# manikya7022/Continual-Learning-for-Dynamic-Video-Quality-Enhancement

Measured on AMD Instinct MI355X. Metric: train frames/sec (2x SR, T=3, 540p->1080p), higher is better.
Workload: dtype bf16

## Files before the change

continual-learning-for-dynamic-video-quality-enhancement_amd/csrc/conv_bf16.hip:

```cpp
#include "conv_common.h"

namespace nvq {

#ifdef NVQ_DEBUG_TOOLS
static int g_debug_mode = 0;
void set_conv_debug_mode(int m) { g_debug_mode = m; }
#else
constexpr int g_debug_mode = 0;
#endif

constexpr int XSB = 48;

__device__ __forceinline__ __bf16 pack_bf16_elem(const float* __restrict__ w, int cout_w, int cin_w, int taps, int transpose,
                                                 int cout_keep, int NT, int nkc, long idx) {
    const int stride = ws_stride_halfs(taps, NT);
    long t = idx % stride;
    const long slab = idx / stride;
    if (t >= (long)taps * 4 * NT * 8) return (__bf16)0.f;
    const int j = t & 7; t >>= 3;
    const int n = t % NT; t /= NT;
    const int g = t & 3; t >>= 2;
    const int tap = (int)t;
    const int kc = slab % nkc;
    const int cz = (int)(slab / nkc);
// ... 721 lines not shown
            for (int k = 0; k < XPER; ++k) {
                const int item = rtid + k * 256;
                *reinterpret_cast<u32x4*>(xs + (item >> 2) * XSB + 8 * (item & 3)) = xok[k] ? xr[k] : z;
            }
        }
        __syncthreads();
        if (kc + 1 < nkc && !(dbg & 4)) fetch(kc + 1);
        if (dbg & 2) continue;
        bf16x8 px[4];
        px[0] = ldP(1, 0, 1); px[1] = ldP(1, 1, 1); px[2] = ldP(2, 0, 1); px[3] = ldP(2, 1, 1);
#pragma unroll
        for (int cb = 0; cb < NBL; ++cb) {
            const bf16x8 wf = ldL(cb);
#pragma unroll
            for (int pb = 0; pb < 4; ++pb)
                lacc[cb][pb] = __builtin_amdgcn_mfma_f32_16x16x32_bf16(wf, px[pb], lacc[cb][pb], 0, 0, 0);
        }
    }
    bool okp[4];
    uint2 rr[4][NBL];
    float4 bb[NBL];
    const __bf16* r16 = reinterpret_cast<const __bf16*>(dl.res) + dl.res_coff;
    auto res_load = [&](int pb) {
        const int gy = ty * TH + 2 * w4 + (pb >> 1), gx = tx * TW + (pb & 1) * 16 + c;
        okp[pb] = gy < H && gx < W;
        const unsigned off = okp[pb] ? ((unsigned)(n * H + gy) * (unsigned)W + gx) * (unsigned)dl.res_ld + 4u * g : 0u;
#pragma unroll
        for (int cb = 0; cb < NBL; ++cb) rr[pb][cb] = *reinterpret_cast<const uint2*>(r16 + (off + cb * 16u));
    };
    if (!(dbg & 128)) { res_load(0); res_load(1); }
    __syncthreads();
    __syncthreads();
    {
        const __bf16* t4 = ws;
#pragma unroll
        for (int cb = 0; cb < NBL; ++cb) {
            const bf16x8 wf = ldL(cb);
#pragma unroll
            for (int pb = 0; pb < 4; ++pb) {
                const int px = (2 * w4 + (pb >> 1)) * TW + (pb & 1) * 16 + c;
                const bf16x8 yf = *reinterpret_cast<const bf16x8*>(t4 + px * T4S + 8 * g);
                lacc[cb][pb] = __builtin_amdgcn_mfma_f32_16x16x32_bf16(wf, yf, lacc[cb][pb], 0, 0, 0);
            }
        }
    }
    if (!(dbg & 128)) { res_load(2); res_load(3); }
#pragma unroll
    for (int cb = 0; cb < NBL; ++cb) bb[cb] = ld4(dl.bias + cb * 16 + 4 * g);
    __syncthreads();
    __bf16* stage = lds + w4 * (2 * TW * STAGE_PX64);
#pragma unroll
    for (int pb = 0; pb < 4; ++pb) {
        if (!okp[pb]) continue;
#pragma unroll
        for (int cb = 0; cb < NBL; ++cb) {
            float v[4] = {lacc[cb][pb][0] + bb[cb].x, lacc[cb][pb][1] + bb[cb].y, lacc[cb][pb][2] + bb[cb].z,
                          lacc[cb][pb][3] + bb[cb].w};
            {
#pragma clang fp contract(off)
                v[0] = v[0] * dl.alpha + __uint_as_float(rr[pb][cb].x << 16);
                v[1] = v[1] * dl.alpha + __uint_as_float(rr[pb][cb].x & 0xffff0000u);
                v[2] = v[2] * dl.alpha + __uint_as_float(rr[pb][cb].y << 16);
                v[3] = v[3] * dl.alpha + __uint_as_float(rr[pb][cb].y & 0xffff0000u);
            }
            *reinterpret_cast<bf16x4*>(stage + ((pb >> 1) * TW + (pb & 1) * 16 + c) * STAGE_PX64 + cb * 16 + 4 * g) =
                (bf16x4){(__bf16)v[0], (__bf16)v[1], (__bf16)v[2], (__bf16)v[3]};
        }
    }
    __builtin_amdgcn_fence(__ATOMIC_RELEASE, "wavefront");
    __builtin_amdgcn_wave_barrier();
    if (dbg & 16) return;
    __bf16* o16 = reinterpret_cast<__bf16*>(dl.out);
#pragma unroll
    for (int k = 0; k < 8; ++k) {
        const int item = lane + k * 64;
        const int px = item >> 3, piece = item & 7;
        const int gy = ty * TH + 2 * w4 + (px >> 5), gx = tx * TW + (px & 31);
        if (gy < H && gx < W)
            *reinterpret_cast<u32x4*>(o16 + ((size_t)(n * H + gy) * W + gx) * dl.out_ld + dl.out_coff + 8 * piece) =
                *reinterpret_cast<const u32x4*>(stage + px * STAGE_PX64 + 8 * piece);
    }
}

template <int KS, bool XB, bool YB, int CIC, int COC = 32>
__global__ __launch_bounds__(256, 2) void wgrad_bf16_kernel(const nvq_wgrad_desc d, int tilesX, int tilesY,
                                                             int ntiles, int nci32, int nco) {
    static_assert(CIC == 32 || (CIC == 64 && XB), "64-channel chunks need bf16 x");
    static_assert(COC == 32 || (COC == 64 && CIC == 64 && YB && KS == 1), "64-co chunks: 1x1, bf16 x and dy");
    constexpr int HALO = KS / 2;
    constexpr int TAPS = KS * KS;
    constexpr int HW_ = TW + 2 * HALO;
    constexpr int HH_ = TH + 2 * HALO;
    constexpr int NPIX = HW_ * HH_;
    constexpr int XSX = CIC == 64 ? 80 : XSB;
    constexpr int XPP = (XB ? 4 : 8) * (CIC / 32);
    constexpr int YSX = COC == 64 ? 80 : XSB;
    constexpr int YPP = (YB ? 4 : 8) * (COC / 32);
    constexpr int XCH = CIC / XPP, YCH = COC / YPP;
    constexpr int XITEMS = NPIX * XPP;
    constexpr int XPER = (XITEMS + 255) / 256;
    constexpr int YPER = TH * TW * YPP / 256;
    constexpr int NCO = (CIC == 64 ? 2 : 1) * (COC / 32);
    __shared__ __attribute__((aligned(16))) __bf16 lds[NPIX * XSX + TH * TW * YSX];
    __bf16* xs = lds;
    __bf16* dys = lds + NPIX * XSX;

    const int tid = threadIdx.x;
    const int lane = tid & 63;
    const int wave = tid >> 6;
    const int r = lane & 15;
    const int g = lane >> 4;
    const int q = r >> 2, p = r & 3;
    const int cib = CIC == 64 ? wave : wave >> 1;
    const int cob0 = CIC == 64 ? 0 : (wave & 1);
    const int cic = blockIdx.y, coc = blockIdx.z;
    const int H = d.h, W = d.w;
    const float* x32 = d.x + d.x_coff;
    const __bf16* x16 = reinterpret_cast<const __bf16*>(d.x) + d.x_coff;
    const float* dy32 = d.dy + d.dy_coff;
    const __bf16* dy16 = reinterpret_cast<const __bf16*>(d.dy) + d.dy_coff;

    f32x4 acc[NCO][TAPS];
#pragma unroll
    for (int a = 0; a < NCO; ++a)
#pragma unroll
        for (int t = 0; t < TAPS; ++t) acc[a][t] = (f32x4){0.f, 0.f, 0.f, 0.f};

    u32x4 xr[XPER], yr[YPER];
    float4 bsumA = make_float4(0.f, 0.f, 0.f, 0.f), bsumB = bsumA;
    const int xq = XCH * (tid & (XPP - 1));
    const int yq = YCH * (tid & (YPP - 1));
    const bool xch_ok = cic * CIC + xq < d.cin;
    const int xch = cic * CIC + xq;
    const bool xlead = !d.x_plane || xch < d.x_ld;
    const unsigned xmul = xlead ? d.x_ld : 32;
    const size_t xbase = xlead ? (size_t)xch : (size_t)(xch >> 5) * d.x_plane + (xch & 31);
    const int ych = coc * COC + yq;
    const bool ych_ok = ych < d.cout;
    unsigned xmask = 0, ymask = 0;
    auto fetch = [&](int tile) {
        int bt = xcd_tile(tile, ntiles);
        const int tx = bt % tilesX; bt /= tilesX;
        const int ty = bt % tilesY;
        const int n = bt / tilesY;
        xmask = 0; ymask = 0;
#pragma unroll
        for (int k = 0; k < XPER; ++k) {
            const int item = tid + k * 256;
            const int hp = item / XPP;
            const int hy = hp / HW_, hx = hp - hy * HW_;
            const int gy = ty * TH + hy - HALO, gx = tx * TW + hx - HALO;
            const bool ok = item < XITEMS && gy >= 0 && gy < H && gx >= 0 && gx < W && xch_ok;
            xmask |= (ok ? 1u : 0u) << k;
            const size_t off = ok ? ((size_t)(n * H + gy) * W + gx) * xmul + xbase : 0;
            if constexpr (XB) xr[k] = *reinterpret_cast<const u32x4*>(x16 + off);
            else xr[k] = *reinterpret_cast<const u32x4*>(x32 + off);
        }
#pragma unroll
        for (int k = 0; k < YPER; ++k) {
            const int item = tid + k * 256;
            const int pp = item / YPP;
            const int py = pp / TW, px = pp - py * TW;
            const int gy = ty * TH + py, gx = tx * TW + px;
            const bool ok = gy < H && gx < W && ych_ok;
            ymask |= (ok ? 1u : 0u) << k;
            const size_t off = ok ? ((size_t)(n * H + gy) * W + gx) * d.dy_ld + ych : 0;
            if constexpr (YB) yr[k] = *reinterpret_cast<const u32x4*>(dy16 + off);
            else yr[k] = *reinterpret_cast<const u32x4*>(dy32 + off);
        }
    };
    auto commit = [&]() {
        const u32x4 z = {0u, 0u, 0u, 0u};
#pragma unroll
        for (int k = 0; k < XPER; ++k) {
            const int item = tid + k * 256;
            if (item < XITEMS) {
                const u32x4 v = (xmask >> k) & 1 ? xr[k] : z;
                __bf16* dst = xs + (item / XPP) * XSX + XCH * (item & (XPP - 1));
                if constexpr (XB) *reinterpret_cast<u32x4*>(dst) = v;
                else *reinterpret_cast<bf16x4*>(dst) = cvt4(as_f4(v));
            }
        }
#pragma unroll
        for (int k = 0; k < YPER; ++k) {
            const int item = tid + k * 256;
            const u32x4 v = (ymask >> k) & 1 ? yr[k] : z;
            __bf16* dst = dys + (item / YPP) * YSX + YCH * (item & (YPP - 1));
            if constexpr (YB) {
                *reinterpret_cast<u32x4*>(dst) = v;
                bsumA.x += bf_lo(v[0]); bsumA.y += bf_hi(v[0]); bsumA.z += bf_lo(v[1]); bsumA.w += bf_hi(v[1]);
                bsumB.x += bf_lo(v[2]); bsumB.y += bf_hi(v[2]); bsumB.z += bf_lo(v[3]); bsumB.w += bf_hi(v[3]);
            } else {
                const float4 f = as_f4(v);
                *reinterpret_cast<bf16x4*>(dst) = cvt4(f);
                bsumA.x += f.x; bsumA.y += f.y; bsumA.z += f.z; bsumA.w += f.w;
            }
        }
    };
    const bool idle = cic * CIC + cib * 16 >= d.cin_w;
    typedef s16x4 __attribute__((address_space(3))) * lds_s16x4_ptr;
    auto tr_read = [&](const __bf16* base, int stride, int pix, int chblock) -> s16x4 {
        return __builtin_amdgcn_ds_read_tr16_b64_v4i16((lds_s16x4_ptr)(base + (pix + q) * stride + chblock * 16 + 4 * p));
    };

    int tile = blockIdx.x;
    if (tile < ntiles) fetch(tile);
    for (; tile < ntiles; tile += gridDim.x) {
        __syncthreads();
        commit();
        __syncthreads();
        if (tile + (int)gridDim.x < ntiles) fetch(tile + gridDim.x);
        if (idle) continue;
#pragma unroll 2
        for (int py = 0; py < TH; ++py) {
            bf16x8 bfrag[NCO];
#pragma unroll
            for (int a = 0; a < NCO; ++a) {
                const s16x4 b0 = tr_read(dys, YSX, py * TW + 4 * g, cob0 + a);
                const s16x4 b1 = tr_read(dys, YSX, py * TW + 16 + 4 * g, cob0 + a);
                bfrag[a] = __builtin_bit_cast(bf16x8, __builtin_shufflevector(b0, b1, 0, 1, 2, 3, 4, 5, 6, 7));
            }
#pragma unroll
            for (int tap = 0; tap < TAPS; ++tap) {
                const int ddy = tap / KS, ddx = tap - ddy * KS;
                const int hp = (py + ddy) * HW_ + ddx;
                const s16x4 a0 = tr_read(xs, XSX, hp + 4 * g, cib);
                const s16x4 a1 = tr_read(xs, XSX, hp + 16 + 4 * g, cib);
                const bf16x8 afrag = __builtin_bit_cast(bf16x8, __builtin_shufflevector(a0, a1, 0, 1, 2, 3, 4, 5, 6, 7));
#pragma unroll
                for (int a = 0; a < NCO; ++a)
                    acc[a][tap] = __builtin_amdgcn_mfma_f32_16x16x32_bf16(afrag, bfrag[a], acc[a][tap], 0, 0, 0);
            }
        }
    }

    const int slab = cic * (CIC / 32) + (cib * 16) / 32;
    if (slab < nci32) {
        const int cil0 = (cib * 16) % 32;
#pragma unroll
        for (int a = 0; a < NCO; ++a) {
            const int coc32 = coc * (COC / 32) + (cob0 + a) / 2, cob = (cob0 + a) % 2;
            if (coc32 >= nco) continue;
            float* part = d.workspace + ((size_t)(blockIdx.x * nci32 + slab) * nco + coc32) * (TAPS * WG_C * WG_C);
#pragma unroll
            for (int tap = 0; tap < TAPS; ++tap)
#pragma unroll
                for (int e = 0; e < 4; ++e) part[(tap * WG_C + cil0 + 4 * g + e) * WG_C + cob * 16 + r] = acc[a][tap][e];
        }
    }

    if (cic == 0 && d.dbias != nullptr) {
        float* scratch = reinterpret_cast<float*>(lds);
        __syncthreads();
        st4(scratch + 8 * tid, bsumA);
        st4(scratch + 8 * tid + 4, bsumB);
        __syncthreads();
        if (tid < COC) {
            const int piece = tid / YCH, e = tid % YCH;
            float s = 0.f;
            for (int k = 0; k < 256 / YPP; ++k) s += scratch[8 * (YPP * k + piece) + e];
            float* bp = d.workspace + (size_t)WGRAD_MAX_SLABS * 9 * WG_C * WG_C;
            const int coc32 = coc * (COC / 32) + tid / WG_C;
            if (coc32 < nco) bp[((size_t)blockIdx.x * nco + coc32) * WG_C + tid % WG_C] = s;
        }
    }
}

size_t pack_floats_bf16(int cout, int cin_store, int ksize) {
    const int NT = choose_nt(cout);
    const size_t ncz = (cout + NT - 1) / NT, nkc = (cin_store + KCB - 1) / KCB;
    return ncz * nkc * (size_t)ws_stride_halfs(ksize * ksize, NT) / 2;
}

int pack_bf16(const float* w, int cout_w, int cin_w, int ksize, int transpose, int cin_store, int cout_keep,
              float* wpack, hipStream_t s) {
    const int cout = transpose ? cout_keep : cout_w;
    const int NT = choose_nt(cout);
    const int ncz = (cout + NT - 1) / NT, nkc = (cin_store + KCB - 1) / KCB;
    const long total = (long)ncz * nkc * ws_stride_halfs(ksize * ksize, NT);
    int nblk = ceil_div(total, 256);
    if (nblk > 2048) nblk = 2048;
    hipLaunchKernelGGL(pack_bf16_kernel, dim3(nblk), dim3(256), 0, s, w, cout_w, cin_w, ksize * ksize, transpose,
                       cout_keep, NT, ncz, nkc, reinterpret_cast<__bf16*>(wpack));
    return check_launch("conv_pack_bf16");
}

PackJobDev pack_job_bf16(const nvq_pack_job& j) {
    const int cout = j.transpose ? j.cout_keep : j.cout_w;
    const int NT = choose_nt(cout);
    const int ncz = (cout + NT - 1) / NT, nkc = (j.cin_store + KCB - 1) / KCB;
    return PackJobDev{j.w, j.wpack, j.cout_w, j.cin_w, j.ksize * j.ksize, j.transpose, j.cout_keep, NT, ncz, nkc,
                      (long)ncz * nkc * ws_stride_halfs(j.ksize * j.ksize, NT)};
}

int pack_batch_bf16(const PackJobTable& t, int n, hipStream_t s) {
    hipLaunchKernelGGL(pack_batch_bf16_kernel, dim3(32, n), dim3(256), 0, s, t);
    return check_launch("conv_pack_batch(bf16)");
}

int conv_forward_bf16(const nvq_conv_desc& d, int vec_ok, hipStream_t s) {
    NVQ_REQUIRE((size_t)d.n * d.h * d.w * d.in_ld < ((size_t)1 << 32),
                "conv_forward(bf16): input tensor of %d x %d x %d x %d elements exceeds the 32-bit offsets of the kernels", d.n,
                d.h, d.w, d.in_ld);
    const int NT = choose_nt(d.cout);
    const int ncz = (d.cout_store + NT - 1) / NT;
    const int nkc = (d.cin + KCB - 1) / KCB;
    int tilesX = (d.w + TW - 1) / TW, tilesY = (d.h + TH - 1) / TH;
    const bool underfilled = tilesX * ((d.h + 2 * TH - 1) / (2 * TH)) < NVQ_SMALL_IMAGE_TILES;
    const int rows = d.tile_rows == 0 && underfilled ? 8 : d.tile_rows;
    if (d.ksize == 3 && NT == 32 && d.in_bf16 && d.h >= 2 * TH && vec_ok &&
        (rows == 162 || rows == 164 || (rows == 0 && d.cin <= 128)))
        return conv_forward_m32(d, rows == 164 ? 4 : 2, g_debug_mode & 15, s);
    if (d.ksize == 3 && NT == 32 && d.in_bf16 && d.h >= 2 * TH && rows != 8) {
        tilesY = (d.h + 2 * TH - 1) / (2 * TH);
        const dim3 grid8((unsigned)((long)tilesX * tilesY * d.n), ncz);
        hipLaunchKernelGGL((conv_bf16_kernel<2, 3, true, 8>), grid8, dim3(512), 0, s, d, tilesX, tilesY, nkc, vec_ok,
                           g_debug_mode & 3, TailArgs{});
        return check_launch("conv_forward_bf16");
    }
    if (d.ksize == 3 && NT == 64 && d.in_bf16 && (d.tile_rows == 264 || d.tile_rows == 265)) {
        NVQ_REQUIRE(vec_ok && d.out_bf16 && d.cout_store % 64 == 0 && d.cin % 8 == 0,
                    "conv_forward: tile_rows 264 / 265 need bf16 output and a multiple of 64 stored channels");
        return conv_forward_m32(d, d.tile_rows == 264 ? 64 : 65, g_debug_mode & 3, s);
    }
    if (d.ksize == 3 && NT == 64 && d.in_bf16 && d.tile_rows != 8) {
        const dim3 grid8((unsigned)((long)tilesX * tilesY * d.n), ncz);
        hipLaunchKernelGGL((conv_bf16_kernel<2, 3, true, 8, 2>), grid8, dim3(512), 0, s, d, tilesX, tilesY, nkc, vec_ok,
                           g_debug_mode & 3, TailArgs{});
        return check_launch("conv_forward_bf16");
    }
    const dim3 grid((unsigned)((long)tilesX * tilesY * d.n), ncz);
#define NVQ_LAUNCH_CONVB(NB, KS)                                                                                        \
    do {                                                                                                                 \
        if (d.in_bf16)                                                                                                   \
            hipLaunchKernelGGL((conv_bf16_kernel<NB, KS, true>), grid, dim3(256), 0, s, d, tilesX, tilesY, nkc, vec_ok, g_debug_mode & 3, TailArgs{});   \
        else                                                                                                             \
            hipLaunchKernelGGL((conv_bf16_kernel<NB, KS, false>), grid, dim3(256), 0, s, d, tilesX, tilesY, nkc, vec_ok, g_debug_mode & 3, TailArgs{});  \
    } while (0)
    if (d.ksize == 3) {
        if (NT == 16) NVQ_LAUNCH_CONVB(1, 3);
        else if (NT == 32) NVQ_LAUNCH_CONVB(2, 3);
        else NVQ_LAUNCH_CONVB(4, 3);
    } else {
        if (NT == 16) NVQ_LAUNCH_CONVB(1, 1);
        else if (NT == 32) NVQ_LAUNCH_CONVB(2, 1);
        else NVQ_LAUNCH_CONVB(4, 1);
    }
#undef NVQ_LAUNCH_CONVB
    return check_launch("conv_forward_bf16");
}

int upsampler_tail_bf16(const nvq_conv_desc& d, const float* frames, int T, int t_center, int Cimg, int s, float* out,
                        unsigned char* pass, hipStream_t st) {
    NVQ_REQUIRE((size_t)d.n * d.h * d.w * d.in_ld < ((size_t)1 << 32), "upsampler_tail: tensor exceeds 32-bit offsets");
    const int tilesX = (d.w + TW - 1) / TW, tilesY = (d.h + TH - 1) / TH;
    const int nkc = (d.cin + KCB - 1) / KCB;
    const dim3 grid((unsigned)((long)tilesX * tilesY * d.n), 1);
    const TailArgs t{frames, out, pass, T, t_center, Cimg};
    if (s == 2 && Cimg * 4 <= 16)
        hipLaunchKernelGGL((conv_bf16_kernel<1, 3, true, 4, 1, 2>), grid, dim3(256), 0, st, d, tilesX, tilesY, nkc, 0, 0, t);
    else if (s == 3 && Cimg * 9 <= 32)
        hipLaunchKernelGGL((conv_bf16_kernel<2, 3, true, 4, 1, 3>), grid, dim3(256), 0, st, d, tilesX, tilesY, nkc, 0, 0, t);
    else if (s == 4 && Cimg * 16 <= 64)
        hipLaunchKernelGGL((conv_bf16_kernel<4, 3, true, 4, 1, 4>), grid, dim3(256), 0, st, d, tilesX, tilesY, nkc, 0, 0, t);
    else
        NVQ_REQUIRE(false, "upsampler_tail: scale %d with %d image channels", s, Cimg);
    return check_launch("upsampler_tail_forward");
}

void conv_occupancy_bf16(int* out) {
    (void)hipOccupancyMaxActiveBlocksPerMultiprocessor(&out[0], conv_bf16_kernel<2, 3, true, 8>, 512, 0);
    (void)hipOccupancyMaxActiveBlocksPerMultiprocessor(&out[1], conv_bf16_kernel<2, 3, true, 8, 2>, 512, 0);
    (void)hipOccupancyMaxActiveBlocksPerMultiprocessor(&out[2], conv_bf16_kernel<4, 3, true, 4>, 256, 0);
    (void)hipOccupancyMaxActiveBlocksPerMultiprocessor(&out[3], rdb_tail_kernel, 256, 0);
    (void)hipOccupancyMaxActiveBlocksPerMultiprocessor(&out[4], wgrad_bf16_kernel<3, true, true, 64, 32>, 256, 0);
    (void)hipOccupancyMaxActiveBlocksPerMultiprocessor(&out[5], conv_bf16_kernel<2, 3, true, 4>, 256, 0);
}

int rdb_tail_bf16(const nvq_conv_desc& d3, const nvq_conv_desc& dl, int vec3, int vecl, hipStream_t s) {
    NVQ_REQUIRE((size_t)d3.n * d3.h * d3.w * d3.in_ld < ((size_t)1 << 32) &&
                    (!dl.res || (size_t)dl.n * dl.h * dl.w * dl.res_ld < ((size_t)1 << 32)),
                "rdb_tail_forward: tensor exceeds 32-bit offsets");
    const int tilesX = (d3.w + TW - 1) / TW, tilesY = (d3.h + TH - 1) / TH;
    const int nkc = d3.cin / KCB;
    const bool usual = dl.out_bf16 && dl.bias && dl.res && dl.res_bf16 && dl.res_cmax >= 64 && !dl.out2 && !dl.relu && vecl;
    if ((d3.tile_rows & 255) == 4 || !usual)
        hipLaunchKernelGGL(rdb_tail_kernel, dim3((unsigned)((long)tilesX * tilesY * d3.n)), dim3(256), 0, s, d3, dl, tilesX,
                           tilesY, nkc, vec3, vecl);
    else
        hipLaunchKernelGGL(rdb_tail8_kernel, dim3((unsigned)((long)tilesX * tilesY * d3.n)), dim3(512), 0, s, d3, dl, tilesX,
                           tilesY, nkc, vec3, vecl);
    return check_launch("rdb_tail_forward");
}

int conv_wgrad_bf16(const nvq_wgrad_desc& d, int nsplit, int nci, int nco, int tilesX, int tilesY, int ntiles,
                    hipStream_t s) {
    if ((d.variant & 15) != 1 && wgrad_m32_takes(d)) return conv_wgrad_m32(d, s);
    NVQ_REQUIRE((d.variant & 15) != 2, "conv_wgrad: variant 2 (all-input-channel kernel) does not take %d -> %d channels, ksize %d",
                d.cin, d.cout, d.ksize);
    const bool wide = d.x_bf16 && d.dy_bf16 && d.cin_w >= 64;
    const int ncig = wide ? (nci + 1) / 2 : nci;
    if (wide) {
        nsplit = WGRAD_MAX_WG / (ncig * nco);
        if (nsplit < 1) nsplit = 1;
        if (nsplit > ntiles) nsplit = ntiles;
        if (nsplit >= 8) nsplit &= ~7;
    }
    NVQ_REQUIRE((size_t)nsplit * nci * nco * d.ksize * d.ksize <= (size_t)WGRAD_MAX_SLABS * 9,
                "conv_wgrad(bf16): %d splits x %d x %d chunks exceed the workspace", nsplit, nci, nco);
    if (wide && d.ksize == 1 && d.cout >= 64) {
        const int nco64 = (nco + 1) / 2;
        nsplit = WGRAD_MAX_WG / (ncig * nco64);
        const int cap = WGRAD_MAX_SLABS * 9 / (nci * nco * d.ksize * d.ksize);
        if (nsplit > cap) nsplit = cap;
        if (nsplit < 1) nsplit = 1;
        if (nsplit > ntiles) nsplit = ntiles;
        if (nsplit >= 8) nsplit &= ~7;
        NVQ_REQUIRE((size_t)nsplit * nci * nco * d.ksize * d.ksize <= (size_t)WGRAD_MAX_SLABS * 9,
                    "conv_wgrad(bf16, 64 co): %d splits x %d x %d chunks exceed the workspace", nsplit, nci, nco);
        hipLaunchKernelGGL((wgrad_bf16_kernel<1, true, true, 64, 64>), dim3(nsplit, ncig, nco64), dim3(256), 0, s, d, tilesX,
                           tilesY, ntiles, nci, nco);
        return nsplit;
    }
    const dim3 grid(nsplit, ncig, nco);
#define NVQ_LAUNCH_WG(KS, XB, YB, CIC) \
    hipLaunchKernelGGL((wgrad_bf16_kernel<KS, XB, YB, CIC>), grid, dim3(256), 0, s, d, tilesX, tilesY, ntiles, nci, nco)
    if (d.ksize == 3) {
        if (wide) NVQ_LAUNCH_WG(3, true, true, 64);
        else if (d.x_bf16 && d.dy_bf16) NVQ_LAUNCH_WG(3, true, true, 32);
        else if (d.x_bf16) NVQ_LAUNCH_WG(3, true, false, 32);
        else if (d.dy_bf16) NVQ_LAUNCH_WG(3, false, true, 32);
        else NVQ_LAUNCH_WG(3, false, false, 32);
    } else {
        if (wide) NVQ_LAUNCH_WG(1, true, true, 64);
        else if (d.x_bf16 && d.dy_bf16) NVQ_LAUNCH_WG(1, true, true, 32);
        else if (d.x_bf16) NVQ_LAUNCH_WG(1, true, false, 32);
        else if (d.dy_bf16) NVQ_LAUNCH_WG(1, false, true, 32);
        else NVQ_LAUNCH_WG(1, false, false, 32);
    }
#undef NVQ_LAUNCH_WG
    return nsplit;
}

}
```

continual-learning-for-dynamic-video-quality-enhancement_amd/csrc/conv_common.h:

```cpp
#pragma once
#include "common.h"

namespace nvq {

constexpr int TH = 8;
constexpr int TW = 32;
constexpr int NVQ_SMALL_IMAGE_TILES = 32;
constexpr int WG_C = 32;
constexpr int WGRAD_MAX_WG = 512;
constexpr int WGRAD_MAX_SLABS = 1536;

static inline int choose_nt(int cout) { return cout <= 16 ? 16 : (cout <= 32 ? 32 : 64); }

#ifdef NVQ_DEBUG_TOOLS
void set_conv_debug_mode(int m);
#endif
void conv_occupancy_bf16(int* out);

typedef short s16x4 __attribute__((ext_vector_type(4)));
typedef unsigned u32x4 __attribute__((ext_vector_type(4)));

constexpr int KCB = 32;

__host__ __device__ constexpr int ws_stride_halfs(int taps, int NT) { return ((taps * 4 * NT * 8 + 2047) / 2048) * 2048; }

__device__ __forceinline__ float4 as_f4(u32x4 v) {
    return make_float4(__uint_as_float(v[0]), __uint_as_float(v[1]), __uint_as_float(v[2]), __uint_as_float(v[3]));
}
__device__ __forceinline__ bf16x4 cvt4(float4 v) {
    return (bf16x4){(__bf16)v.x, (__bf16)v.y, (__bf16)v.z, (__bf16)v.w};
}
__device__ __forceinline__ bf16x8 cvt8(float4 a, float4 b) {
    return (bf16x8){(__bf16)a.x, (__bf16)a.y, (__bf16)a.z, (__bf16)a.w, (__bf16)b.x, (__bf16)b.y, (__bf16)b.z, (__bf16)b.w};
}
__device__ __forceinline__ float bf_lo(unsigned u) { return __uint_as_float(u << 16); }
__device__ __forceinline__ float bf_hi(unsigned u) { return __uint_as_float(u & 0xffff0000u); }

size_t pack_floats_bf16(int cout, int cin_store, int ksize);
int pack_bf16(const float* w, int cout_w, int cin_w, int ksize, int transpose, int cin_store, int cout_keep,
              float* wpack, hipStream_t s);
struct PackJobDev { const float* w; float* wp; int cout_w, cin_w, taps, transpose, cout_keep, NT, ncz, nkc; long total; };
constexpr int PACK_BATCH = 48;
struct PackJobTable { PackJobDev j[PACK_BATCH]; };
int pack_batch_bf16(const PackJobTable& t, int n, hipStream_t s);
PackJobDev pack_job_bf16(const nvq_pack_job& j);
int conv_forward_bf16(const nvq_conv_desc& d, int vec_ok, hipStream_t s);
int conv_wgrad_bf16(const nvq_wgrad_desc& d, int nsplit, int nci, int nco, int tilesX, int tilesY, int ntiles,
                    hipStream_t s);
int upsampler_tail_bf16(const nvq_conv_desc& d, const float* frames, int T, int t_center, int Cimg, int s, float* out,
                        unsigned char* pass, hipStream_t st);
int rdb_tail_bf16(const nvq_conv_desc& d3, const nvq_conv_desc& dl, int vec3, int vecl, hipStream_t s);
int conv_forward_m32(const nvq_conv_desc& d, int variant, int dbg, hipStream_t s);
void conv_occupancy_m32(int* out);
bool wgrad_m32_takes(const nvq_wgrad_desc& d);
int conv_wgrad_m32(const nvq_wgrad_desc& d, hipStream_t s);

__device__ __forceinline__ void wgrad_bias_partial(const nvq_wgrad_desc& d, float4 bsum, float* lds, int nco, int cic,
                                                   int coc) {
    if (cic != 0 || d.dbias == nullptr) return;
    __syncthreads();
    st4(lds + 4 * threadIdx.x, bsum);
    __syncthreads();
    if (threadIdx.x < 32) {
        const int q = threadIdx.x >> 2, e = threadIdx.x & 3;
        float s = 0.f;
        for (int k = 0; k < 32; ++k) s += lds[4 * (8 * k + q) + e];
        float* bp = d.workspace + (size_t)WGRAD_MAX_SLABS * 9 * WG_C * WG_C;
        bp[((size_t)blockIdx.x * nco + coc) * WG_C + threadIdx.x] = s;
    }
}

constexpr int STAGE_PX = 40;
constexpr int STAGE_PX64 = 72;

typedef unsigned raw4 __attribute__((ext_vector_type(4)));
__device__ __forceinline__ raw4 ld_raw4(const float* base, size_t idx, int is_bf16) {
    raw4 r;
    if (is_bf16) {
        const uint2 t = *reinterpret_cast<const uint2*>(reinterpret_cast<const __bf16*>(base) + idx);
        r[0] = t.x; r[1] = t.y;
    } else {
        r = *reinterpret_cast<const raw4*>(base + idx);
    }
    return r;
}
__device__ __forceinline__ float4 raw4_f(raw4 r, int is_bf16) {
    if (is_bf16)
        return make_float4(__uint_as_float(r[0] << 16), __uint_as_float(r[0] & 0xffff0000u), __uint_as_float(r[1] << 16),
                           __uint_as_float(r[1] & 0xffff0000u));
    return make_float4(__uint_as_float(r[0]), __uint_as_float(r[1]), __uint_as_float(r[2]), __uint_as_float(r[3]));
}

template <int NB, bool FULL = (NB <= 2)>
__device__ __forceinline__ void conv_epilogue(const nvq_conv_desc& d, f32x4 (&acc)[NB][4], int n, int ty, int tx,
                                              int cz, int wave, int c, int g, int vec_ok, int th = TH,
                                              __bf16* stage = nullptr, int stage_px = STAGE_PX, bool barrier = false) {
    constexpr int NT = NB * 16;
    const int H = d.h, W = d.w;
    if (vec_ok) {
        bool okp[4];
        size_t pixv[4];
#pragma unroll
        for (int pb = 0; pb < 4; ++pb) {
            const int gy = ty * th + 2 * wave + (pb >> 1), gx = tx * TW + (pb & 1) * 16 + c;
            okp[pb] = gy < H && gx < W;
            pixv[pb] = okp[pb] ? (size_t)(n * H + gy) * W + gx : 0;
        }
        int cov[NB];
#pragma unroll
        for (int cb = 0; cb < NB; ++cb) cov[cb] = cz * NT + cb * 16 + 4 * g;
        constexpr int CG = FULL ? NB : 1;
        constexpr int RP = FULL ? 4 : 1;
        float4 bias4[CG];
        unsigned bits_in[4];
        raw4 res4[CG][RP], msk4[CG];
        auto bias_load = [&](int cb0) {
#pragma unroll
            for (int k = 0; k < CG; ++k) bias4[k] = ld4(d.bias + (cov[cb0 + k] < d.cout ? cov[cb0 + k] : 0));
        };
        auto res_load = [&](int pb, int cb0, int slot) {
#pragma unroll
            for (int k = 0; k < CG; ++k)
                res4[k][slot] = ld_raw4(d.res, pixv[pb] * d.res_ld + d.res_coff + (cov[cb0 + k] < d.res_cmax ? cov[cb0 + k] : 0),
                                        d.res_bf16);
        };
        const int bw = d.bits_words > 0 ? d.bits_words : 1, wsel = (cz * NT) >> 5;
        if constexpr (NB <= 2) {
            if (d.bits_mode == 2) {
#pragma unroll
                for (int pb = 0; pb < 4; ++pb) bits_in[pb] = d.bits[pixv[pb] * bw + wsel];
            }
        }
        if constexpr (FULL) {
            if (d.bias) bias_load(0);
            if (d.res) {
#pragma unroll
                for (int pb = 0; pb < 4; ++pb) res_load(pb, 0, pb);
            }
        }
        if (barrier) __syncthreads();
#pragma unroll
        for (int pb = 0; pb < 4; ++pb) {
            if (!okp[pb]) continue;
            const size_t pix = pixv[pb];
            unsigned bits_out = 0;
#pragma unroll
            for (int cb = 0; cb < NB; ++cb) {
                const int k = cb % CG;
                if (k == 0) {
                    if constexpr (!FULL) {
                        if (d.bias) bias_load(cb);
                        if (d.res) res_load(pb, cb, 0);
                    }
                    if (d.mask) {
#pragma unroll
                        for (int j = 0; j < CG; ++j) {
                            const bool in = cov[cb + j] >= d.mask_c0 && cov[cb + j] < d.mask_c1;
                            msk4[j] = ld_raw4(d.mask, pix * d.mask_ld + d.mask_coff + (in ? cov[cb + j] : 0), d.mask_bf16);
                        }
                    }
                }
                const int co = cov[cb];
                if (co >= d.cout_store) continue;
                float v[4] = {acc[cb][pb][0], acc[cb][pb][1], acc[cb][pb][2], acc[cb][pb][3]};
                if (d.bias && co < d.cout) {
                    v[0] += bias4[k].x; v[1] += bias4[k].y; v[2] += bias4[k].z; v[3] += bias4[k].w;
                }
                if (d.relu) {
#pragma unroll
                    for (int e = 0; e < 4; ++e) v[e] = fmaxf(v[e], 0.f);
                }
#pragma unroll
                for (int e = 0; e < 4; ++e) v[e] *= d.alpha;
                if (d.out2)
                    stx4(d.out2, pix * d.out2_ld + d.out2_coff + co, d.out2_bf16, make_float4(v[0], v[1], v[2], v[3]));
                if (d.res && co < d.res_cmax) {
                    const float4 r = raw4_f(res4[k][RP == 4 ? pb : 0], d.res_bf16);
                    v[0] += r.x; v[1] += r.y; v[2] += r.z; v[3] += r.w;
                }
                const size_t oi = pix * d.out_ld + d.out_coff + co;
                if (d.accumulate) {
                    const float4 o = ldx4(d.out, oi, d.out_bf16);
                    v[0] += o.x; v[1] += o.y; v[2] += o.z; v[3] += o.w;
                }
                if (d.mask && co >= d.mask_c0 && co < d.mask_c1) {
                    const float4 m = raw4_f(msk4[k], d.mask_bf16);
                    if (!(m.x > 0.f)) v[0] = 0.f;
                    if (!(m.y > 0.f)) v[1] = 0.f;
                    if (!(m.z > 0.f)) v[2] = 0.f;
                    if (!(m.w > 0.f)) v[3] = 0.f;
                }
                if constexpr (NB <= 2) {
                    if (d.bits_mode == 2) {
#pragma unroll
                        for (int e = 0; e < 4; ++e)
                            if (!((bits_in[pb] >> ((co & 31) + e)) & 1u)) v[e] = 0.f;
                    } else if (d.bits_mode == 1) {
#pragma unroll
                        for (int e = 0; e < 4; ++e) bits_out |= (v[e] > 0.f ? 1u : 0u) << ((co & 31) + e);
                    }
                }
                if (stage)
                    *reinterpret_cast<bf16x4*>(stage + ((pb >> 1) * TW + (pb & 1) * 16 + c) * stage_px + co - cz * NT) =
                        (bf16x4){(__bf16)v[0], (__bf16)v[1], (__bf16)v[2], (__bf16)v[3]};
                else
                    stx4(d.out, oi, d.out_bf16, make_float4(v[0], v[1], v[2], v[3]));
            }
            if constexpr (NB <= 2) {
                if (d.bits_mode == 1) {
                    bits_out |= __shfl_xor(bits_out, 16, 64);
                    bits_out |= __shfl_xor(bits_out, 32, 64);
                    if (g == 0) d.bits[pix * bw + wsel] = bits_out;
                }
            }
        }
        return;
    }
#pragma unroll
    for (int pb = 0; pb < 4; ++pb) {
        const int row = 2 * wave + (pb >> 1);
        const int gy = ty * th + row;
        const int gx = tx * TW + (pb & 1) * 16 + c;
        if (gy >= H || gx >= W) continue;
        const size_t pix = (size_t)(n * H + gy) * W + gx;
#pragma unroll
        for (int cb = 0; cb < NB; ++cb) {
            const int co = cz * NT + cb * 16 + 4 * g;
#pragma unroll
            for (int e = 0; e < 4; ++e) {
                const int ce = co + e;
                if (ce >= d.cout_store) continue;
                float x = acc[cb][pb][e];
                if (d.bias && ce < d.cout) x += d.bias[ce];
                if (d.relu) x = fmaxf(x, 0.f);
                x *= d.alpha;
                if (d.out2) d.out2[pix * d.out2_ld + d.out2_coff + ce] = x;
                if (d.res && ce < d.res_cmax) x += d.res[pix * d.res_ld + d.res_coff + ce];
                float* op = d.out + pix * d.out_ld + d.out_coff + ce;
                if (d.accumulate) x += *op;
                if (d.mask && ce >= d.mask_c0 && ce < d.mask_c1 &&
                    !(d.mask[pix * d.mask_ld + d.mask_coff + ce] > 0.f))
                    x = 0.f;
                *op = x;
            }
        }
    }
}

}
```

Measured before the change: 79.60.

## Add narrow-channel conv forward and wgrad kernels for few-channel layers

Adds dedicated kernels for 3x3 convolutions with very few input channels (up to 12, e.g. the RGB/frame input layer) in the forward pass, and for weight gradients where one side has few channels. The forward kernel packs taps times channel groups into the MFMA K dimension instead of padding each tap to 32 channels, and keeps the weights in registers. The wgrad kernel uses a persistent tile loop with prefetching and transposed LDS reads. This is meant to cut the wasted MFMA work and memory traffic that the general kernels spend on zero-padded channels, at the cost of extra code paths and some register pressure.

New measurement: 80.39 (median of 6 runs). Within noise of the previous version (+1.0%).

```diff
diff --git a/continual-learning-for-dynamic-video-quality-enhancement_amd/csrc/conv_bf16.hip b/continual-learning-for-dynamic-video-quality-enhancement_amd/csrc/conv_bf16.hip
--- a/continual-learning-for-dynamic-video-quality-enhancement_amd/csrc/conv_bf16.hip
+++ b/continual-learning-for-dynamic-video-quality-enhancement_amd/csrc/conv_bf16.hip
@@ -1047,6 +1047,7 @@
     NVQ_REQUIRE((size_t)d.n * d.h * d.w * d.in_ld < ((size_t)1 << 32),
                 "conv_forward(bf16): input tensor of %d x %d x %d x %d elements exceeds the 32-bit offsets of the kernels", d.n,
                 d.h, d.w, d.in_ld);
+    if (conv_narrow_takes(d)) return conv_forward_narrow(d, vec_ok, s);
     const int NT = choose_nt(d.cout);
     const int ncz = (d.cout_store + NT - 1) / NT;
     const int nkc = (d.cin + KCB - 1) / KCB;
@@ -1141,6 +1142,7 @@
 int conv_wgrad_bf16(const nvq_wgrad_desc& d, int nsplit, int nci, int nco, int tilesX, int tilesY, int ntiles,
                     hipStream_t s) {
     if ((d.variant & 15) != 1 && wgrad_m32_takes(d)) return conv_wgrad_m32(d, s);
+    if (wgrad_narrow_takes(d)) return conv_wgrad_narrow(d, tilesX, tilesY, ntiles, s);
     NVQ_REQUIRE((d.variant & 15) != 2, "conv_wgrad: variant 2 (all-input-channel kernel) does not take %d -> %d channels, ksize %d",
                 d.cin, d.cout, d.ksize);
     const bool wide = d.x_bf16 && d.dy_bf16 && d.cin_w >= 64;
diff --git a/continual-learning-for-dynamic-video-quality-enhancement_amd/csrc/conv_common.h b/continual-learning-for-dynamic-video-quality-enhancement_amd/csrc/conv_common.h
--- a/continual-learning-for-dynamic-video-quality-enhancement_amd/csrc/conv_common.h
+++ b/continual-learning-for-dynamic-video-quality-enhancement_amd/csrc/conv_common.h
@@ -52,6 +52,10 @@
 int rdb_tail_bf16(const nvq_conv_desc& d3, const nvq_conv_desc& dl, int vec3, int vecl, hipStream_t s);
 int conv_forward_m32(const nvq_conv_desc& d, int variant, int dbg, hipStream_t s);
 void conv_occupancy_m32(int* out);
+bool conv_narrow_takes(const nvq_conv_desc& d);
+int conv_forward_narrow(const nvq_conv_desc& d, int vec_ok, hipStream_t s);
+bool wgrad_narrow_takes(const nvq_wgrad_desc& d);
+int conv_wgrad_narrow(const nvq_wgrad_desc& d, int tilesX, int tilesY, int ntiles, hipStream_t s);
 bool wgrad_m32_takes(const nvq_wgrad_desc& d);
 int conv_wgrad_m32(const nvq_wgrad_desc& d, hipStream_t s);
 
diff --git a/continual-learning-for-dynamic-video-quality-enhancement_amd/csrc/conv_narrow.hip b/continual-learning-for-dynamic-video-quality-enhancement_amd/csrc/conv_narrow.hip
--- /dev/null
+++ b/continual-learning-for-dynamic-video-quality-enhancement_amd/csrc/conv_narrow.hip
@@ -0,0 +1,392 @@
+#include "conv_common.h"
+
+namespace nvq {
+
+constexpr int XSB_W = 48;
+constexpr int NARROW_TILE_ROWS = 12;
+
+template <int NB, int CG>
+__global__ __launch_bounds__(256, NB * ((9 * CG + 7) / 8) > 8 ? 3 : 4) void conv_narrow_kernel(const nvq_conv_desc d, int tilesX,
+                                                                                              int tilesY, int vec_ok) {
+    constexpr int NT = NB * 16;
+    constexpr int NW = 4, TH_ = 2 * NW;
+    constexpr int HW_ = TW + 2, HH_ = TH_ + 2, NPIX = HW_ * HH_;
+    constexpr int PXH = CG * 4;
+    constexpr int NPC = 9 * CG;
+    constexpr int KSTEPS = (NPC + 7) / 8;
+    constexpr int XITEMS = NPIX * CG;
+    constexpr int XPER = (XITEMS + 255) / 256;
+    constexpr int WS_HALFS = ws_stride_halfs(9, NT);
+    constexpr int SPX = NB == 2 ? STAGE_PX : STAGE_PX64;
+    static_assert(NB == 2 || NB == 4, "32 or 64 output channels per workgroup");
+
+    __shared__ __attribute__((aligned(16))) __bf16 xs[NPIX * PXH];
+    __shared__ __attribute__((aligned(16))) __bf16 stg[NW * 2 * TW * SPX];
+
+    const int tid = threadIdx.x;
+    const int lane = tid & 63;
+    const int wave = __builtin_amdgcn_readfirstlane(tid >> 6);
+    const int c = lane & 15;
+    const int g = lane >> 4;
+    const int cz = blockIdx.y;
+    const int H = d.h, W = d.w;
+    const float* in32 = d.in + d.in_coff;
+
+    int boff[KSTEPS][2];
+    bool bval[KSTEPS][2];
+    bf16x8 a[NB][KSTEPS];
+    {
+        const __bf16* wp = reinterpret_cast<const __bf16*>(d.wpack) + (size_t)cz * WS_HALFS;
+        const bf16x4 z4 = {(__bf16)0.f, (__bf16)0.f, (__bf16)0.f, (__bf16)0.f};
+#pragma unroll
+        for (int s = 0; s < KSTEPS; ++s) {
+            bf16x4 ap[NB][2];
+#pragma unroll
+            for (int j = 0; j < 2; ++j) {
+                const int q = 8 * s + 2 * g + j;
+                const bool v = q < NPC;
+                const int tap = v ? q / CG : 0, grp = v ? q - tap * CG : 0;
+                const int dy = tap / 3, dx = tap - dy * 3;
+                bval[s][j] = v;
+                boff[s][j] = ((dy * HW_ + dx) * CG + grp) * 4;
+#pragma unroll
+                for (int cb = 0; cb < NB; ++cb) {
+                    const bf16x4 w4 = *reinterpret_cast<const bf16x4*>(wp + ((tap * 4 + (grp >> 1)) * NT + cb * 16 + c) * 8 + (grp & 1) * 4);
+                    ap[cb][j] = v ? w4 : z4;
+                }
+            }
+#pragma unroll
+            for (int cb = 0; cb < NB; ++cb) a[cb][s] = __builtin_shufflevector(ap[cb][0], ap[cb][1], 0, 1, 2, 3, 4, 5, 6, 7);
+        }
+    }
+
+    int bt = xcd_tile(blockIdx.x, gridDim.x);
+    const int tx = bt % tilesX; bt /= tilesX;
+    const int ty = bt % tilesY;
+    const int n = bt / tilesY;
+
+    unsigned warm = 0;
+    if (vec_ok) {
+        const int gy = ty * TH_ + 2 * wave + (lane >> 5), gx = tx * TW + (lane & 31);
+        const size_t pix = gy < H && gx < W ? (size_t)(n * H + gy) * W + gx : 0;
+        if (d.bits_mode == 2) warm ^= d.bits[pix * (d.bits_words > 0 ? d.bits_words : 1) + ((cz * NT) >> 5)];
+        if (d.mask) {
+            const int mc = cz * NT > d.mask_c0 ? cz * NT : d.mask_c0;
+            const size_t e = pix * d.mask_ld + d.mask_coff + (mc < d.mask_c1 ? mc : 0);
+            warm ^= *reinterpret_cast<const unsigned*>(reinterpret_cast<const char*>(d.mask) + e * (d.mask_bf16 ? 2 : 4));
+        }
+        if (d.res) {
+            const size_t e = pix * d.res_ld + d.res_coff + (cz * NT < d.res_cmax ? cz * NT : 0);
+            warm ^= *reinterpret_cast<const unsigned*>(reinterpret_cast<const char*>(d.res) + e * (d.res_bf16 ? 2 : 4));
+        }
+    }
+
+    {
+        u32x4 xr[XPER];
+        bool xok[XPER];
+#pragma unroll
+        for (int k = 0; k < XPER; ++k) {
+            const int item = tid + k * 256;
+            const int hp = item / CG, grp = item - hp * CG;
+            const int hy = hp / HW_, hx = hp - hy * HW_;
+            const int gy = ty * TH_ + hy - 1, gx = tx * TW + hx - 1;
+            xok[k] = item < XITEMS && gy >= 0 && gy < H && gx >= 0 && gx < W;
+            const unsigned off = xok[k] ? (unsigned)(((size_t)(n * H + gy) * W + gx) * d.in_ld) + 4 * grp : 0u;
+            xr[k] = *reinterpret_cast<const u32x4*>(in32 + off);
+        }
+        const u32x4 z = {0u, 0u, 0u, 0u};
+#pragma unroll
+        for (int k = 0; k < XPER; ++k) {
+            const int item = tid + k * 256;
+            if (item < XITEMS) *reinterpret_cast<bf16x4*>(xs + item * 4) = cvt4(as_f4(xok[k] ? xr[k] : z));
+        }
+    }
+    __syncthreads();
+    {
+        f32x4 acc[NB][4];
+#pragma unroll
+        for (int cb = 0; cb < NB; ++cb)
+#pragma unroll
+            for (int pb = 0; pb < 4; ++pb) acc[cb][pb] = (f32x4){0.f, 0.f, 0.f, 0.f};
+        const bf16x4 z4 = {(__bf16)0.f, (__bf16)0.f, (__bf16)0.f, (__bf16)0.f};
+#pragma unroll
+        for (int pb = 0; pb < 4; ++pb) {
+            const __bf16* px = xs + ((2 * wave + (pb >> 1)) * HW_ + (pb & 1) * 16 + c) * PXH;
+#pragma unroll
+            for (int s = 0; s < KSTEPS; ++s) {
+                bf16x4 p0 = *reinterpret_cast<const bf16x4*>(px + boff[s][0]);
+                bf16x4 p1 = *reinterpret_cast<const bf16x4*>(px + boff[s][1]);
+                if (8 * s + 8 > NPC) {
+                    p0 = bval[s][0] ? p0 : z4;
+                    p1 = bval[s][1] ? p1 : z4;
+                }
+                const bf16x8 b = __builtin_shufflevector(p0, p1, 0, 1, 2, 3, 4, 5, 6, 7);
+#pragma unroll
+                for (int cb = 0; cb < NB; ++cb) acc[cb][pb] = __builtin_amdgcn_mfma_f32_16x16x32_bf16(a[cb][s], b, acc[cb][pb], 0, 0, 0);
+            }
+        }
+
+        asm volatile("" ::"v"(warm));
+
+        if (d.out_bf16 && vec_ok && d.cout_store - cz * NT >= NT) {
+            constexpr int PPP = NT / 8;
+            __bf16* stage = stg + wave * (2 * TW * SPX);
+            conv_epilogue<NB>(d, acc, n, ty, tx, cz, wave, c, g, vec_ok, TH_, stage, SPX, false);
+            __builtin_amdgcn_fence(__ATOMIC_RELEASE, "wavefront");
+            __builtin_amdgcn_wave_barrier();
+            __bf16* o16 = reinterpret_cast<__bf16*>(d.out);
+#pragma unroll
+            for (int k = 0; k < PPP; ++k) {
+                const int item = lane + k * 64;
+                const int p = item / PPP, piece = item % PPP;
+                const int gy = ty * TH_ + 2 * wave + (p >> 5), gx = tx * TW + (p & 31);
+                if (gy < H && gx < W)
+                    *reinterpret_cast<u32x4*>(o16 + ((size_t)(n * H + gy) * W + gx) * d.out_ld + d.out_coff + cz * NT + 8 * piece) =
+                        *reinterpret_cast<const u32x4*>(stage + p * SPX + 8 * piece);
+            }
+        } else {
+            conv_epilogue<NB>(d, acc, n, ty, tx, cz, wave, c, g, vec_ok, TH_);
+        }
+    }
+}
+
+bool conv_narrow_takes(const nvq_conv_desc& d) {
+    return d.ksize == 3 && !d.in_bf16 && d.in_plane == 0 && d.center_cin == 0 && d.cin <= 12 && choose_nt(d.cout) >= 32 &&
+           (d.tile_rows == 0 || d.tile_rows == NARROW_TILE_ROWS);
+}
+
+int conv_forward_narrow(const nvq_conv_desc& d, int vec_ok, hipStream_t s) {
+    const int NT = choose_nt(d.cout);
+    const int ncz = (d.cout_store + NT - 1) / NT;
+    const int tilesX = (d.w + TW - 1) / TW, tilesY = (d.h + TH - 1) / TH;
+    const long ntiles = (long)tilesX * tilesY * d.n;
+    NVQ_REQUIRE(ntiles < (1L << 31), "conv_forward(narrow): %ld tiles", ntiles);
+    const dim3 grid((unsigned)ntiles, ncz);
+    const int cg = d.cin / 4;
+#define NVQ_LAUNCH_NARROW(NB, CG) \
+    hipLaunchKernelGGL((conv_narrow_kernel<NB, CG>), grid, dim3(256), 0, s, d, tilesX, tilesY, vec_ok)
+    if (NT == 32) {
+        if (cg == 1) NVQ_LAUNCH_NARROW(2, 1);
+        else if (cg == 2) NVQ_LAUNCH_NARROW(2, 2);
+        else NVQ_LAUNCH_NARROW(2, 3);
+    } else {
+        if (cg == 1) NVQ_LAUNCH_NARROW(4, 1);
+        else if (cg == 2) NVQ_LAUNCH_NARROW(4, 2);
+        else NVQ_LAUNCH_NARROW(4, 3);
+    }
+#undef NVQ_LAUNCH_NARROW
+    return check_launch("conv_forward_narrow");
+}
+
+template <int CIC, int CG, bool SWAP = false>
+__global__ __launch_bounds__(256, 2) void wgrad_narrow_co_kernel(const nvq_wgrad_desc d, int tilesX, int tilesY, int ntiles) {
+    static_assert(!SWAP || CG == 1, "narrow input: one 4-channel group");
+    constexpr int CO4 = 4 * CG;
+    constexpr int HWd = TW + 2, HHd = TH + 2, NPIXD = HWd * HHd;
+    constexpr int XSX = CIC == 64 ? 80 : XSB_W;
+    constexpr int XPP = 4 * (CIC / 32);
+    constexpr int PPT = 256 / CG;
+    constexpr int DR = (NPIXD + PPT - 1) / PPT;
+    constexpr int NCIB = CIC / 16, NWN = 4 / NCIB;
+    constexpr int NNB = (9 * CG + 3) / 4;
+    constexpr int NJ = (NNB + NWN - 1) / NWN;
+    constexpr int SLAB = 9 * WG_C * WG_C;
+    __shared__ __attribute__((aligned(16))) __bf16 lds[TH * TW * XSX + NPIXD * CO4 + 8];
+    __bf16* xs = lds;
+    __bf16* dys = lds + TH * TW * XSX;
+    static_assert((TH * TW * XSX + NPIXD * CO4) * 2 >= 256 * 8 * 4, "the bias partials reuse the stages");
+
+    const int tid = threadIdx.x;
+    const int lane = tid & 63;
+    const int wave = __builtin_amdgcn_readfirstlane(tid >> 6);
+    const int r = lane & 15, g = lane >> 4;
+    const int q = r >> 2, p = r & 3;
+    const int cib = wave % NCIB, nsel = wave / NCIB;
+    const int H = d.h, W = d.w;
+    const __bf16* x16 = SWAP ? reinterpret_cast<const __bf16*>(d.dy) + d.dy_coff : reinterpret_cast<const __bf16*>(d.x) + d.x_coff;
+    const float* dy32 = d.dy + d.dy_coff;
+    const __bf16* nx16 = reinterpret_cast<const __bf16*>(d.x) + d.x_coff;
+    const int wide_ld = SWAP ? d.dy_ld : d.x_ld;
+
+    f32x4 acc[NJ];
+    int boff[NJ];
+#pragma unroll
+    for (int j = 0; j < NJ; ++j) {
+        acc[j] = (f32x4){0.f, 0.f, 0.f, 0.f};
+        const int nq = (nsel + NWN * j) * 4 + p;
+        const bool v = nq < 9 * CG;
+        const int tap = v ? nq / CG : 0, grp = v ? nq - tap * CG : 0;
+        const int ddy = tap / 3, ddx = tap - ddy * 3;
+        boff[j] = SWAP ? (ddy * HWd + ddx + q) * CO4 + 4 * grp : ((2 - ddy) * HWd + (2 - ddx) + q) * CO4 + 4 * grp;
+    }
+
+    const int xq = 8 * (tid & (XPP - 1));
+    const int ygrp = tid % CG, ypx = tid / CG;
+    const bool yact = tid < PPT * CG;
+    u32x4 xr[XPP], yr[DR];
+    unsigned xmask = 0, ymask = 0, bmask = 0;
+    float4 bsum = make_float4(0.f, 0.f, 0.f, 0.f);
+    float4 bsumB = bsum;
+    auto fetch = [&](int tile) {
+        int bt = xcd_tile(tile, ntiles);
+        const int tx = bt % tilesX; bt /= tilesX;
+        const int ty = bt % tilesY;
+        const int n = bt / tilesY;
+        xmask = 0; ymask = 0; bmask = 0;
+#pragma unroll
+        for (int k = 0; k < XPP; ++k) {
+            const int pp = (tid + k * 256) / XPP;
+            const int py = pp / TW, px = pp - py * TW;
+            const int gy = ty * TH + py, gx = tx * TW + px;
+            const bool ok = gy < H && gx < W;
+            xmask |= (ok ? 1u : 0u) << k;
+            const size_t off = ok ? ((size_t)(n * H + gy) * W + gx) * wide_ld + xq : 0;
+            xr[k] = *reinterpret_cast<const u32x4*>(x16 + off);
+        }
+#pragma unroll
+        for (int k = 0; k < DR; ++k) {
+            const int hp = k * PPT + ypx;
+            const int hy = hp / HWd, hx = hp - hy * HWd;
+            const int gy = ty * TH + hy - 1, gx = tx * TW + hx - 1;
+            const bool ok = yact && hp < NPIXD && gy >= 0 && gy < H && gx >= 0 && gx < W;
+            ymask |= (ok ? 1u : 0u) << k;
+            bmask |= (ok && hy >= 1 && hy <= TH && hx >= 1 && hx <= TW ? 1u : 0u) << k;
+            if constexpr (SWAP) {
+                const uint2 t = *reinterpret_cast<const uint2*>(nx16 + (ok ? ((size_t)(n * H + gy) * W + gx) * d.x_ld : 0));
+                yr[k] = (u32x4){t.x, t.y, 0u, 0u};
+            } else {
+                const size_t off = ok ? ((size_t)(n * H + gy) * W + gx) * d.dy_ld + 4 * ygrp : 0;
+                yr[k] = *reinterpret_cast<const u32x4*>(dy32 + off);
+            }
+        }
+    };
+    auto commit = [&]() {
+        const u32x4 z = {0u, 0u, 0u, 0u};
+#pragma unroll
+        for (int k = 0; k < XPP; ++k) {
+            const int item = tid + k * 256;
+            const u32x4 v = (xmask >> k) & 1 ? xr[k] : z;
+            *reinterpret_cast<u32x4*>(xs + (item / XPP) * XSX + xq) = v;
+            if constexpr (SWAP) {
+                bsum.x += bf_lo(v[0]); bsum.y += bf_hi(v[0]); bsum.z += bf_lo(v[1]); bsum.w += bf_hi(v[1]);
+                bsumB.x += bf_lo(v[2]); bsumB.y += bf_hi(v[2]); bsumB.z += bf_lo(v[3]); bsumB.w += bf_hi(v[3]);
+            }
+        }
+#pragma unroll
+        for (int k = 0; k < DR; ++k) {
+            const int hp = k * PPT + ypx;
+            const u32x4 v = (ymask >> k) & 1 ? yr[k] : z;
+            if constexpr (SWAP) {
+                if (hp < NPIXD) *reinterpret_cast<uint2*>(dys + hp * CO4) = make_uint2(v[0], v[1]);
+            } else {
+                const float4 f = as_f4(v);
+                if (yact && hp < NPIXD) *reinterpret_cast<bf16x4*>(dys + hp * CO4 + 4 * ygrp) = cvt4(f);
+                if ((bmask >> k) & 1) { bsum.x += f.x; bsum.y += f.y; bsum.z += f.z; bsum.w += f.w; }
+            }
+        }
+    };
+    typedef s16x4 __attribute__((address_space(3))) * lds_s16x4_ptr;
+
+    int tile = blockIdx.x;
+    if (tile < ntiles) fetch(tile);
+    for (; tile < ntiles; tile += gridDim.x) {
+        __syncthreads();
+        commit();
+        __syncthreads();
+        if (tile + (int)gridDim.x < ntiles) fetch(tile + gridDim.x);
+#pragma unroll 2
+        for (int py = 0; py < TH; ++py) {
+            const __bf16* xa = xs + (py * TW + 4 * g + q) * XSX + cib * 16 + 4 * p;
+            const s16x4 a0 = __builtin_amdgcn_ds_read_tr16_b64_v4i16((lds_s16x4_ptr)xa);
+            const s16x4 a1 = __builtin_amdgcn_ds_read_tr16_b64_v4i16((lds_s16x4_ptr)(xa + 16 * XSX));
+            const bf16x8 afrag = __builtin_bit_cast(bf16x8, __builtin_shufflevector(a0, a1, 0, 1, 2, 3, 4, 5, 6, 7));
+            const __bf16* yb = dys + (py * HWd + 4 * g) * CO4;
+#pragma unroll
+            for (int j = 0; j < NJ; ++j) {
+                if (nsel + NWN * j >= NNB) continue;
+                const s16x4 b0 = __builtin_amdgcn_ds_read_tr16_b64_v4i16((lds_s16x4_ptr)(yb + boff[j]));
+                const s16x4 b1 = __builtin_amdgcn_ds_read_tr16_b64_v4i16((lds_s16x4_ptr)(yb + boff[j] + 16 * CO4));
+                const bf16x8 bfrag = __builtin_bit_cast(bf16x8, __builtin_shufflevector(b0, b1, 0, 1, 2, 3, 4, 5, 6, 7));
+                acc[j] = __builtin_amdgcn_mfma_f32_16x16x32_bf16(afrag, bfrag, acc[j], 0, 0, 0);
+            }
+        }
+    }
+
+    {
+        const int ci = cib * 16 + 4 * g;
+        float* part = d.workspace + ((size_t)blockIdx.x * (CIC / 32) + ci / 32) * SLAB;
+#pragma unroll
+        for (int j = 0; j < NJ; ++j) {
+            const int n = (nsel + NWN * j) * 16 + r;
+            if (nsel + NWN * j >= NNB || n >= 9 * CO4) continue;
+            const int tap = n / CO4, co = n - tap * CO4;
+#pragma unroll
+            for (int e = 0; e < 4; ++e) {
+                if constexpr (SWAP) part[(tap * WG_C + co) * WG_C + (ci & 31) + e] = acc[j][e];
+                else part[(tap * WG_C + (ci & 31) + e) * WG_C + co] = acc[j][e];
+            }
+        }
+    }
+    if (d.dbias != nullptr) {
+        float* scratch = reinterpret_cast<float*>(lds);
+        __syncthreads();
+        if constexpr (SWAP) {
+            st4(scratch + 8 * tid, bsum);
+            st4(scratch + 8 * tid + 4, bsumB);
+        } else {
+            st4(scratch + 4 * tid, bsum);
+        }
+        __syncthreads();
+        float* bpw = d.workspace + (size_t)WGRAD_MAX_SLABS * 9 * WG_C * WG_C;
+        if constexpr (SWAP) {
+            if (tid < CIC) {
+                float s = 0.f;
+                for (int k = 0; k < 256 / XPP; ++k) s += scratch[8 * (XPP * k + tid / 8) + (tid & 7)];
+                bpw[(size_t)blockIdx.x * CIC + tid] = s;
+            }
+        } else if (tid < CO4) {
+            const int grp = tid >> 2, e = tid & 3;
+            float s = 0.f;
+            for (int k = 0; k < PPT; ++k) s += scratch[4 * (k * CG + grp) + e];
+            float* bp = d.workspace + (size_t)WGRAD_MAX_SLABS * 9 * WG_C * WG_C;
+            bp[(size_t)blockIdx.x * WG_C + tid] = s;
+        }
+    }
+}
+
+static bool wgrad_narrow_ci(const nvq_wgrad_desc& d) {
+    return d.ksize == 3 && d.x_bf16 && d.dy_bf16 && d.x_plane == 0 && d.cin_w <= 4 && (d.cout == 32 || d.cout == 64);
+}
+
+bool wgrad_narrow_takes(const nvq_wgrad_desc& d) {
+    if ((d.variant & 15) != 0) return false;
+    if (wgrad_narrow_ci(d)) return true;
+    return d.ksize == 3 && d.x_bf16 && !d.dy_bf16 && d.x_plane == 0 && d.cout <= 12 &&
+           (d.cin == 32 || d.cin == 64) && (d.cin_w + WG_C - 1) / WG_C == d.cin / WG_C;
+}
+
+int conv_wgrad_narrow(const nvq_wgrad_desc& d, int tilesX, int tilesY, int ntiles, hipStream_t s) {
+    int nsplit = WGRAD_MAX_WG < ntiles ? WGRAD_MAX_WG : ntiles;
+    if (nsplit >= 8) nsplit &= ~7;
+    const int cg = (d.cout + 3) / 4;
+    const dim3 grid(nsplit);
+    if (wgrad_narrow_ci(d)) {
+        if (d.cout == 32) hipLaunchKernelGGL((wgrad_narrow_co_kernel<32, 1, true>), grid, dim3(256), 0, s, d, tilesX, tilesY, ntiles);
+        else hipLaunchKernelGGL((wgrad_narrow_co_kernel<64, 1, true>), grid, dim3(256), 0, s, d, tilesX, tilesY, ntiles);
+        return nsplit;
+    }
+#define NVQ_LAUNCH_WN(CIC, CG) hipLaunchKernelGGL((wgrad_narrow_co_kernel<CIC, CG>), grid, dim3(256), 0, s, d, tilesX, tilesY, ntiles)
+    if (d.cin == 32) {
+        if (cg == 1) NVQ_LAUNCH_WN(32, 1);
+        else if (cg == 2) NVQ_LAUNCH_WN(32, 2);
+        else NVQ_LAUNCH_WN(32, 3);
+    } else {
+        if (cg == 1) NVQ_LAUNCH_WN(64, 1);
+        else if (cg == 2) NVQ_LAUNCH_WN(64, 2);
+        else NVQ_LAUNCH_WN(64, 3);
+    }
+#undef NVQ_LAUNCH_WN
+    return nsplit;
+}
+
+}
```
